# mprib/caliscope

Hardware: AMD Instinct MI355X
Metric: observations/sec per LM iteration (higher is better)
Workload: dtype f64; 1 GPU; cfg4: 64 cams / 2000000 obs in total (200000 points / 2000000 obs on rank 0), extrinsics-only BA, linear loss; n_obs_total=2000000, params_per_camera=6, tolerances=ftol=xtol=gtol=1e-8 (reference defaults), sums=FP64 atomics (default)

## Files before the change

caliscope_amd/csrc/ba_math.h:

```cpp
#pragma once
#include <cstddef>
#include <cmath>
#include <cstdint>

#if defined(__HIPCC__)
#define CBA_HD __host__ __device__ __forceinline__
#else
#define CBA_HD inline
#endif

namespace cba {

constexpr int MODEL_PINHOLE_BC5 = 0;
constexpr int MODEL_FISHEYE4 = 1;
constexpr int CAM_CONST_STRIDE = 12;
constexpr int MAX_NC = 9;
constexpr double EPS_F64 = 2.220446049250313e-16;

CBA_HD double inv_sqrt(double x) {
#if defined(__HIP_DEVICE_COMPILE__)
  double y = __builtin_amdgcn_rsq(x);
  y = y * (1.5 - 0.5 * x * y * y);
  y = y * (1.5 - 0.5 * x * y * y);
  return y;
// ... 134 lines not shown
  const double g10 = fys * L.dyx * iz, g11 = fys * L.dyy * iz;
  const double G[2][3] = {{g00, g01, -(g00 * x + g01 * y)}, {g10, g11, -(g10 * x + g11 * y)}};
  for (int r = 0; r < 2; ++r) {
    A[r][3] = G[r][0]; A[r][4] = G[r][1]; A[r][5] = G[r][2];
    B[r][0] = G[r][0] * c.R[0] + G[r][1] * c.R[3] + G[r][2] * c.R[6];
    B[r][1] = G[r][0] * c.R[1] + G[r][1] * c.R[4] + G[r][2] * c.R[7];
    B[r][2] = G[r][0] * c.R[2] + G[r][1] * c.R[5] + G[r][2] * c.R[8];
  }
  for (int j = 0; j < 3; ++j) {
    const double m0 = c.Jl[j], m1 = c.Jl[3 + j], m2 = c.Jl[6 + j];
    const double c0 = m1 * Y2 - m2 * Y1, c1 = m2 * Y0 - m0 * Y2, c2 = m0 * Y1 - m1 * Y0;
    A[0][j] = G[0][0] * c0 + G[0][1] * c1 + G[0][2] * c2;
    A[1][j] = G[1][0] * c0 + G[1][1] * c1 + G[1][2] * c2;
  }
  if (c.nparams == 9.0) {
    A[0][6] = c.fx0 * L.xd * s; A[1][6] = c.fy0 * L.yd * s;
    A[0][7] = fxs * L.xr2;      A[1][7] = fys * L.yr2;
    A[0][8] = fxs * L.xr4;      A[1][8] = fys * L.yr4;
  }
}

template <bool RES>
CBA_HD void project_factors_impl(const CamTab& c, double X, double Y, double Z, double u, double v,
                                 double* e, double (*G)[3], double* Yr, double (*Aint)[3], double (*B)[3]) {
  const double Y0 = c.R[0] * X + c.R[1] * Y + c.R[2] * Z;
  const double Y1 = c.R[3] * X + c.R[4] * Y + c.R[5] * Z;
  const double Y2 = c.R[6] * X + c.R[7] * Y + c.R[8] * Z;
  Yr[0] = Y0; Yr[1] = Y1; Yr[2] = Y2;
  const double Zc = Y2 + c.t[2];
  const double iz = 1.0 / Zc;
  const double x = (Y0 + c.t[0]) * iz, y = (Y1 + c.t[1]) * iz;
  Lens L;
  if (c.model != 0.0) lens_fisheye(c.d, x, y, &L); else lens_pinhole(c.d, x, y, &L);
  const double s = c.inv_fx0;
  if constexpr (RES) {
    e[0] = ((c.cx - u) + c.fx * L.xd) * s;
    e[1] = ((c.cy - v) + c.fy * L.yd) * s;
  }
  const double fxs = c.fx * s, fys = c.fy * s;
  const double g00 = fxs * L.dxx * iz, g01 = fxs * L.dxy * iz;
  const double g10 = fys * L.dyx * iz, g11 = fys * L.dyy * iz;
  G[0][0] = g00; G[0][1] = g01; G[0][2] = -(g00 * x + g01 * y);
  G[1][0] = g10; G[1][1] = g11; G[1][2] = -(g10 * x + g11 * y);
  for (int r = 0; r < 2; ++r) {
    B[r][0] = G[r][0] * c.R[0] + G[r][1] * c.R[3] + G[r][2] * c.R[6];
    B[r][1] = G[r][0] * c.R[1] + G[r][1] * c.R[4] + G[r][2] * c.R[7];
    B[r][2] = G[r][0] * c.R[2] + G[r][1] * c.R[5] + G[r][2] * c.R[8];
  }
  const bool free_intr = c.nparams == 9.0;
  Aint[0][0] = free_intr ? c.fx0 * L.xd * s : 0.0; Aint[1][0] = free_intr ? c.fy0 * L.yd * s : 0.0;
  Aint[0][1] = free_intr ? fxs * L.xr2 : 0.0;      Aint[1][1] = free_intr ? fys * L.yr2 : 0.0;
  Aint[0][2] = free_intr ? fxs * L.xr4 : 0.0;      Aint[1][2] = free_intr ? fys * L.yr4 : 0.0;
}
CBA_HD void project_factors(const CamTab& c, double X, double Y, double Z, double u, double v,
                            double* e, double (*G)[3], double* Yr, double (*Aint)[3], double (*B)[3]) {
  project_factors_impl<true>(c, X, Y, Z, u, v, e, G, Yr, Aint, B);
}
CBA_HD void project_factors(const CamTab& c, double X, double Y, double Z, double (*G)[3], double* Yr, double (*Aint)[3], double (*B)[3]) {
  project_factors_impl<false>(c, X, Y, Z, 0.0, 0.0, nullptr, G, Yr, Aint, B);
}

CBA_HD double robust_one(int loss, double f_scale, double r, double* row_scale, double* r_scaled) {
  if (loss == LOSS_LINEAR) { *row_scale = 1.0; *r_scaled = r; return r * r; }
  const double fs2 = f_scale * f_scale;
  const double z = (r * r) / fs2;
  double rho0, rho1, rho2;
  switch (loss) {
    case LOSS_HUBER:
      if (z <= 1.0) { rho0 = z; rho1 = 1.0; rho2 = 0.0; }
      else { const double sz = sqrt(z); rho0 = 2.0 * sz - 1.0; rho1 = 1.0 / sz; rho2 = -0.5 / (z * sz); }
      break;
    case LOSS_SOFT_L1: {
      const double t = 1.0 + z, st = sqrt(t);
      rho0 = 2.0 * (st - 1.0); rho1 = 1.0 / st; rho2 = -0.5 / (t * st);
    } break;
    case LOSS_CAUCHY: {
      const double t = 1.0 + z;
      rho0 = log1p(z); rho1 = 1.0 / t; rho2 = -1.0 / (t * t);
    } break;
    default: {
      const double t = 1.0 + z * z;
      rho0 = atan(z); rho1 = 1.0 / t; rho2 = -2.0 * z / (t * t);
// ... 158 lines not shown
```

caliscope_amd/csrc/cba_kernels.h:

```cpp
#pragma once
#include <hip/hip_runtime.h>

#include "ba_math.h"
#include "trf_math.h"
#include "wg_binding.h"
#include "chol_schedule.h"

namespace cba {

constexpr int BLOCK = 256;
constexpr int CHUNK = 256;
constexpr int WAVE = 64;

struct VecLayout {
  int ncp;
  int ncp_pad;
  int P;
  int Ppad;
  __host__ __device__ long total() const { return (long)ncp_pad + 3L * Ppad; }
};

__device__ __forceinline__ double wave_sum(double v) {
#pragma unroll
  for (int o = WAVE / 2; o > 0; o >>= 1) v += __shfl_down(v, o, WAVE);
// ... 290 lines not shown
template <int NC>
__device__ __forceinline__ double obs_linearize(const CamTab& c_lds, double X, double Y, double Z, double u, double v,
                                                int loss, double f_scale, double* e, double (*A)[MAX_NC],
                                                double (*B)[3]) {
  const CamTab c = c_lds;
  __builtin_amdgcn_sched_barrier(0);
  project_full(c, X, Y, Z, u, v, e, A, B);
  double rho = 0.0;
#pragma unroll
  for (int r = 0; r < 2; ++r) {
    double rs, er;
    rho += robust_one(loss, f_scale, e[r], &rs, &er);
    e[r] = er;
    if (loss != LOSS_LINEAR) {
#pragma unroll
      for (int k = 0; k < NC; ++k) A[r][k] *= rs;
      B[r][0] *= rs; B[r][1] *= rs; B[r][2] *= rs;
    }
  }
  return rho;
}

__device__ __forceinline__ double obs_factors(const CamTab& c_lds, double X, double Y, double Z, double u, double v, int loss, double f_scale, double* e,
                                              double (*G)[3], double* Yr, double (*Aint)[3], double (*B)[3]) {
  CamTab c;
  {
    const double* src = reinterpret_cast<const double*>(&c_lds);
    double* dst = reinterpret_cast<double*>(&c);
#pragma unroll
    for (int i = 0; i < 12; ++i) dst[i] = src[i];
#pragma unroll
    for (int i = 21; i < 35; ++i) dst[i] = src[i];
  }
  __builtin_amdgcn_sched_barrier(0);
  project_factors(c, X, Y, Z, u, v, e, G, Yr, Aint, B);
  double rho = 0.0;
#pragma unroll
  for (int r = 0; r < 2; ++r) {
    double rs, er;
    rho += robust_one(loss, f_scale, e[r], &rs, &er);
    e[r] = er;
    if (loss != LOSS_LINEAR) {
#pragma unroll
      for (int k = 0; k < 3; ++k) { G[r][k] *= rs; B[r][k] *= rs; Aint[r][k] *= rs; }
    }
  }
  return rho;
}
__device__ __forceinline__ void obs_factors(const CamTab& c_lds, double X, double Y, double Z, double (*G)[3], double* Yr, double (*Aint)[3], double (*B)[3]) {
  CamTab c;
  {
    const double* src = reinterpret_cast<const double*>(&c_lds);
    double* dst = reinterpret_cast<double*>(&c);
#pragma unroll
    for (int i = 0; i < 12; ++i) dst[i] = src[i];
    dst[21] = src[21]; dst[22] = src[22];
#pragma unroll
    for (int i = 25; i < 35; ++i) dst[i] = src[i];
  }
  __builtin_amdgcn_sched_barrier(0);
  project_factors(c, X, Y, Z, G, Yr, Aint, B);
#pragma unroll
  for (int r = 0; r < 2; ++r) {
#pragma unroll
    for (int k = 0; k < 3; ++k) { asm("" : "+v"(G[r][k])); asm("" : "+v"(B[r][k])); asm("" : "+v"(Aint[r][k])); }
  }
#pragma unroll
  for (int k = 0; k < 3; ++k) asm("" : "+v"(Yr[k]));
}

template <int NC> struct UPack {
  static constexpr int TRI = NC * (NC + 1) / 2;
  static constexpr int STRIDE = TRI + NC;
  __host__ __device__ static constexpr int idx(int r, int c) { return r * NC - r * (r - 1) / 2 + (c - r); }
};

constexpr int DET_ROUND = 9;
constexpr int DET_LD = CHUNK + 1;
struct DetPlan {
  const unsigned char* perm;
  const unsigned short* cstart;
};
template <int M>
__device__ __forceinline__ void det_round(const double* val, double* sh_cv, const int* sh_perm, const int* sh_cs, int n_cams, double* acc) {
#pragma unroll
  for (int q = 0; q < DET_ROUND; ++q) sh_cv[q * DET_LD + threadIdx.x] = val[q];
  __syncthreads();
#pragma unroll
  for (int m = 0; m < M; ++m) {
    const int task = (int)threadIdx.x + BLOCK * m;
    if (task < n_cams * DET_ROUND) {
// ... 585 lines not shown
}

struct TilePlan {
  const int* chunk_start;
  const int* wg_first;
  const int* wg_end;
  const int* wg_tile;
  const int* wg_stride;
  const int* tile_a;
  const int* tile_b;
  const int* group_cam_begin;
  const int* group_par_begin;
  int g;
  int tile_elems;
  const int* obs;
  int rep;
  const unsigned* codes;
  const int* code_start;
  const unsigned* nit;
  int prio_shift;
};

template <int NC> struct SchurRec {
  static constexpr int NVAL = (NC == 9) ? 21 : 12;
  static constexpr int NPH = (NVAL + 1) / 2;
  static constexpr int LST = (NPH & 1) ? NPH : NPH + 1;
  static constexpr int REC = 2 * LST;
  static constexpr int HREC = 2 * NPH;
  static constexpr int STAGE = (HREC / 2) | 1;
  static constexpr int STAGE_WAVES = (NC == 9) ? 2 : 4;
};
static_assert(SchurRec<6>::REC == 14 && SchurRec<6>::LST == 7 && SchurRec<9>::REC == 22 && SchurRec<9>::LST == 11, "record sizes");

template <int NC>
__device__ __forceinline__ void expand_record(const double* __restrict__ rec, const double* __restrict__ Jl, double* __restrict__ T) {
  const double Y0 = rec[0], Y1 = rec[1], Y2 = rec[2];
  const double* Q = rec + 3;
#pragma unroll
  for (int m = 0; m < 3; ++m) {
    const double q0 = Q[m], q1 = Q[3 + m], q2 = Q[6 + m];
    const double c0 = Y1 * q2 - Y2 * q1, c1 = Y2 * q0 - Y0 * q2, c2 = Y0 * q1 - Y1 * q0;
#pragma unroll
    for (int r = 0; r < 3; ++r) T[3 * r + m] = Jl[r] * c0 + Jl[3 + r] * c1 + Jl[6 + r] * c2;
    T[9 + m] = q0; T[12 + m] = q1; T[15 + m] = q2;
  }
  if (NC == 9) {
#pragma unroll
    for (int k = 0; k < 9; ++k) T[18 + k] = rec[12 + k];
  }
}

struct LinFin {
  const double* partial_lin;
  const double* partial_max;
  const double* partial_jv;
  int rows_lin, rows_jv;
  double radius;
  double* scal;
  double* fz;
};
// ... 143 lines not shown
      const int k1 = min(no0 + (int)threadIdx.x, last_obs);
      if constexpr (!LIN) { nx.u = obs_u[k1]; nx.v = obs_v[k1]; }
      nx.cam = obs_cam[k1];
      nn.pt = obs_pt[min(nno0 + (int)threadIdx.x, last_obs)];
    } else {
      nn = load_rec(min((PIPE ? nno0 : no0) + (int)threadIdx.x, last_obs));
    }
    if constexpr (PIPE) __builtin_amdgcn_sched_barrier(0);
    const int i = o0 + threadIdx.x;
    double rec[REC];
#pragma unroll
    for (int k = 0; k < REC; ++k) rec[k] = 0.0;
    double bval[DET_ROUND];
#pragma unroll
    for (int q = 0; q < DET_ROUND; ++q) bval[q] = 0.0;
    if (DET) {
      sh_perm[threadIdx.x] = det.perm[(long)ch * CHUNK + threadIdx.x];
      for (int q = threadIdx.x; q <= n_cams; q += BLOCK) sh_cs[q] = det.cstart[(long)ch * (n_cams + 1) + q];
    }
    if (i < o1) {
      const int cam = cur.cam;
      const CamTab& ct = cam_of<CAMG>(sh_tab, tab, cam);
      const double X = ops.X, Yw = ops.Y, Zw = ops.Z;
      double e[2], G[2][3], Yr[3], Aint[2][3], B[2][3], Z[2][3];
      if constexpr (LIN) obs_factors(ct, X, Yw, Zw, G, Yr, Aint, B);
      else obs_factors(ct, X, Yw, Zw, cur.u, cur.v, loss, f_scale, e, G, Yr, Aint, B);
      const int np = (int)ct.nparams;
      double Vd[6], L[6];
#pragma unroll
      for (int q = 0; q < 6; ++q) Vd[q] = ops.V[q];
      const double d0 = ops.d[0], d1 = ops.d[1], d2 = ops.d[2];
      Vd[0] += lam * d0 * d0; Vd[3] += lam * d1 * d1; Vd[5] += lam * d2 * d2;
      if (!chol3(Vd, L)) {
        fail = true;
        L[0] = L[2] = L[5] = 1.0; L[1] = L[3] = L[4] = 0.0;
      }
      chol3_fwd(L, B[0], Z[0]);
      chol3_fwd(L, B[1], Z[1]);
      const double gpt[3] = {ops.g[0], ops.g[1], ops.g[2]};
      double y[3];
      chol3_fwd(L, gpt, y);
      double* bc = sh_b + (int)ct.pad[0];
      rec[0] = Yr[0]; rec[1] = Yr[1]; rec[2] = Yr[2];
      double qy[3];
#pragma unroll
      for (int r = 3; r < NC; ++r) {
        const bool live = r < np;
        const double a0 = (r < 6) ? G[0][r - 3] : Aint[0][(r - 6) % 3], a1 = (r < 6) ? G[1][r - 3] : Aint[1][(r - 6) % 3];
        double t[3];
#pragma unroll
        for (int k = 0; k < 3; ++k) t[k] = live ? a0 * Z[0][k] + a1 * Z[1][k] : 0.0;
        const double ty = t[0] * y[0] + t[1] * y[1] + t[2] * y[2];
        if (r < 6) qy[r - 3] = ty;
        if (DET) bval[r] = live ? ty : 0.0;
        else if (live) lds_add(&bc[r], ty);
        rec[3 * r - 6] = t[0]; rec[3 * r - 5] = t[1]; rec[3 * r - 4] = t[2];
      }
      {
        const double c0 = Yr[1] * qy[2] - Yr[2] * qy[1], c1 = Yr[2] * qy[0] - Yr[0] * qy[2], c2 = Yr[0] * qy[1] - Yr[1] * qy[0];
        if (DET) {
#pragma unroll
          for (int r = 0; r < 3; ++r) bval[r] = ct.Jl[r] * c0 + ct.Jl[3 + r] * c1 + ct.Jl[6 + r] * c2;
        } else {
          lds_add(&bc[0], c0); lds_add(&bc[1], c1); lds_add(&bc[2], c2);
        }
      }
    }
    if constexpr (PIPE) {
      asm volatile("s_waitcnt vmcnt(0)" ::: "memory");
      if constexpr (FULL) launder_obs(nn); else { launder_obs(nx); asm volatile("" : "+v"(nn.pt)); }
      launder_ops(ops_n);
    }
    const int w0 = o0 + wv * WAVE;
    const int n_pieces = max(0, min(WAVE, o1 - w0)) * NP;
    double2* dst = reinterpret_cast<double2*>(Trec + (long)w0 * REC);
#pragma unroll
    for (int turn = 0; turn < (BLOCK / WAVE) / SW; ++turn) {
      if (wv / SW == turn) {
#pragma unroll
// ... 115 lines not shown
  static constexpr int SPLIT = (NC == 9) ? 3 : 1;
  static constexpr int CODE_THREADS = BLOCK, CODE_WAVES = BLOCK / WAVE;
  static constexpr int REG_BLOCK = BLOCK * SPLIT, NWAVES = REG_BLOCK / WAVE;
  static constexpr int GROUP = 16;
  static constexpr int NCD = (NC == 6) ? 8 : 4;
  static constexpr int PAIR_CAP = 0;
  static constexpr int SCHUNK = (NC == 9) ? 384 : 320;
  static constexpr int EPW = SCHUNK / NWAVES;
  static constexpr int NLD = (EPW * LST + WAVE - 1) / WAVE;
  static constexpr int WAVE_PIECES = NLD * WAVE;
  static constexpr int ZERO_PIECE = NWAVES * WAVE_PIECES;
  static constexpr int BUF_PIECES = ZERO_PIECE + LST + 1;
  static constexpr int NBUF = 2;
  static constexpr int SET_PIECES = NBUF * BUF_PIECES;
  static constexpr bool LANE_TABLE = (NC == 9);
  static constexpr int TABLE_PIECES = LANE_TABLE ? (NLD * WAVE * 4 + 15) / 16 : 0;
  static constexpr size_t LDS_BYTES = (size_t)(SET_PIECES + TABLE_PIECES) * 16;
  static constexpr int LAUNCH_THREADS = REG_BLOCK;
  static_assert(SCHUNK % NWAVES == 0 && EPW % 16 == 0 && EPW <= 2 * WAVE && (LST & 1) == 1, "staging layout");
  static_assert(ZERO_PIECE + LST < 65536, "piece addresses are 16 bit");
  static_assert(CODE_WAVES % 4 == 0, "iteration counts: four waves per word");
};

__device__ __forceinline__ void pair6(double (&acc)[6][6], const double2* __restrict__ Ri, const double2* __restrict__ Rj) {
  const double2 i0 = Ri[0], i1 = Ri[1], i2 = Ri[2], i3 = Ri[3], i4 = Ri[4], i5 = Ri[5];
  const double2 j0 = Rj[0], j1 = Rj[1], j2 = Rj[2], j3 = Rj[3], j4 = Rj[4], j5 = Rj[5];
  const double Yi[3] = {i0.x, i0.y, i1.x}, Yj[3] = {j0.x, j0.y, j1.x};
  const double Qi[9] = {i1.y, i2.x, i2.y, i3.x, i3.y, i4.x, i4.y, i5.x, i5.y};
  const double Qj[9] = {j1.y, j2.x, j2.y, j3.x, j3.y, j4.x, j4.y, j5.x, j5.y};
  double M[3][6];
#pragma unroll
  for (int a = 0; a < 3; ++a) {
#pragma unroll
    for (int b2 = 0; b2 < 3; ++b2)
      M[a][3 + b2] = fma(Qi[3 * a + 2], Qj[3 * b2 + 2], fma(Qi[3 * a + 1], Qj[3 * b2 + 1], Qi[3 * a] * Qj[3 * b2]));
    M[a][0] = fma(Yj[1], M[a][5], -(Yj[2] * M[a][4]));
    M[a][1] = fma(Yj[2], M[a][3], -(Yj[0] * M[a][5]));
    M[a][2] = fma(Yj[0], M[a][4], -(Yj[1] * M[a][3]));
  }
#pragma unroll
  for (int c = 0; c < 6; ++c) {
    acc[0][c] = fma(Yi[1], M[2][c], fma(-Yi[2], M[1][c], acc[0][c]));
    acc[1][c] = fma(Yi[2], M[0][c], fma(-Yi[0], M[2][c], acc[1][c]));
    acc[2][c] = fma(Yi[0], M[1][c], fma(-Yi[1], M[0][c], acc[2][c]));
    acc[3][c] += M[0][c]; acc[4][c] += M[1][c]; acc[5][c] += M[2][c];
  }
}

template <int NC, int RH>
__device__ __forceinline__ void unprime_rows(double (&acc)[RH][NC], int r0, const double* __restrict__ Ji, const double* __restrict__ Jj) {
  if (r0 == 0) {
#pragma unroll
    for (int c = 0; c < NC; ++c) {
      const double b0 = acc[0][c], b1 = acc[1][c], b2 = acc[2][c];
#pragma unroll
      for (int r = 0; r < 3; ++r) acc[r][c] = Ji[r] * b0 + Ji[3 + r] * b1 + Ji[6 + r] * b2;
    }
  }
// ... 32 lines not shown
    for (int c = 0; c < 6; ++c) acc[r][c] = 0.0;

  const int vt = (SPLIT == 1) ? tid : ct;
  const int blk = (rep > 1) ? vt % nblk : vt, slot = (rep > 1) ? vt / nblk : 0;
  const bool owner = slot < rep && blk < nblk;
  double* dst = partial + ((long)wg * rep + min(slot, rep - 1)) * tp.tile_elems + (long)min(blk, nblk - 1) * NC * NC;

  const int stride = tp.wg_stride[wg], ch_end = tp.wg_end[wg];
  const int own_trips = tp.wg_first[wg] < ch_end ? (ch_end - 1 - tp.wg_first[wg]) / stride + 1 : 0;
  const int first = own_trips ? tp.wg_first[wg] : max(ch_end - 1, 0);
  const int trips = max(own_trips, 1);
  for (int k = tid; k < Cfg::NBUF * LST; k += REG_BLOCK) sh_p[(k / LST) * Cfg::BUF_PIECES + Cfg::ZERO_PIECE + k % LST] = make_double2(0.0, 0.0);
  int* const lane_table = reinterpret_cast<int*>(sh_p + Cfg::SET_PIECES);
  if constexpr (Cfg::LANE_TABLE) {
    constexpr int Q = WAVE / LST, RM = WAVE % LST;
    for (int e = tid; e < NLD * WAVE; e += REG_BLOCK) {
      const int k = e / WAVE, l = e % WAVE;
      int piece = k * RM + l % LST;
      const int el = min(k * Q + l / LST + piece / LST, EPW - 1);
      piece = min(piece % LST, SchurRec<NC>::NPH - 1);
      lane_table[e] = el | (piece << 16);
    }
    __syncthreads();
  }
  const int last = first + (own_trips ? (own_trips - 1) * stride : 0);
  struct Raw { unsigned nit[NWORD]; int code_start; int obs_start; };
  auto load_raw = [&](int chunk, int successor) {
    Raw r;
#pragma unroll
    for (int q = 0; q < NWORD; ++q) r.nit[q] = p_nit[(long)chunk * NWORD + q];
    r.code_start = p_code_start[chunk];
    r.obs_start = p_chunk_start[successor];
    return r;
  };
  auto load_indices = [&](int obs_start, int* iA, int* iB) {
    const int* src = p_obs + obs_start + sw * EPW;
    *iA = src[lane];
    if (EPW > WAVE) *iB = src[WAVE + (lane & (EPW - WAVE - 1))];
  };
  static_assert(EPW <= WAVE || ((EPW - WAVE) & (EPW - WAVE - 1)) == 0, "second index register");
  unsigned cd[NCD];
  int n_nx = 0;
  long code_nx = 0;
  auto load_codes = [&](const Raw& r) {
    int pre = 0, mine = 0;
#pragma unroll
// ... 19 lines not shown
      int piece, el;
      if constexpr (Cfg::LANE_TABLE) {
        const int e = lane_table[k * WAVE + lane];
        el = e & 0xffff; piece = e >> 16;
      } else {
        piece = k * RM + lane % LST;
        el = k * Q + lane / LST + piece / LST;
        piece = min(piece % LST, SchurRec<NC>::NPH - 1);
        el = min(el, EPW - 1);
      }
      const bool useB = EPW > WAVE && k * WAVE >= WAVE * LST;
      const int idx = useB ? __shfl(idxB, el - WAVE, WAVE) : __shfl(idxA, el, WAVE);
      g[k] = reinterpret_cast<const double2*>(Trec + (long)idx * SchurRec<NC>::HREC) + piece;
    }
    __builtin_amdgcn_sched_barrier(0);
#pragma unroll
    for (int k = 0; k < NLD; ++k)
      __builtin_amdgcn_global_load_lds((const void __attribute__((address_space(1)))*)g[k], (void __attribute__((address_space(3)))*)(wbase + k * WAVE), 16, 0, 0);
  };
  auto pair = [&](const double2* bufp, unsigned code) {
    const double2* Ri = bufp + (code & 0xffffu);
    const double2* Rj = bufp + (code >> 16);
    if constexpr (NC == 6) {
      pair6(acc, Ri, Rj);
    } else {
      if (half == 0) pair9_corner(acc, Ri, Rj);
      else if (half == 1) pair9_cols(accf, Ri, Rj);
      else pair9_rows(accf, Ri, Rj);
    }
  };

  long long clk_sum[6] = {0, 0, 0, 0, 0, 0};
  const long long t_start = CLK ? clock64() : 0;
  int idxA = 0, idxB = 0;
  const int second = min(first + stride, last);
  Raw raw = load_raw(first, second);
  load_indices(p_chunk_start[first], &idxA, &idxB);
  issue(0, idxA, idxB);
  load_codes(raw);
  load_indices(raw.obs_start, &idxA, &idxB);
  raw = load_raw(second, min(second + stride, last));
  int buf = 0;
  const int young = ((int)blockIdx.x >= (int)gridDim.x / 2) ? 1 : 0;
  for (int trip = 0; trip < trips; ++trip) {
    if (tp.prio_shift >= 0) {
      if (((trip >> tp.prio_shift) + young) & 1) __builtin_amdgcn_s_setprio(1); else __builtin_amdgcn_s_setprio(0);
    }
// ... 26 lines not shown
    __builtin_amdgcn_sched_barrier(0);
    if (CLK) { tD = clock64(); __builtin_amdgcn_sched_barrier(0); }
    const double2* bufp = sh_p + buf * Cfg::BUF_PIECES;
#pragma unroll
    for (int it = 0; it < NCD; ++it)
      if (it < n_cur) pair(bufp, cc[it]);
    for (int it = NCD; it < n_cur; ++it) pair(bufp, p_codes[code_cur + (long)it * WAVE]);
    if (CLK) {
      __builtin_amdgcn_sched_barrier(0);
      const long long tE = clock64();
      clk_sum[0] += tB - tA; clk_sum[1] += tC - tB; clk_sum[2] += tD - tC; clk_sum[3] += tE - tD; clk_sum[4] += 1; clk_sum[5] += n_cur;
    }
    raw = raw_n; idxA = idxA_n; idxB = idxB_n;
    buf ^= 1;
  }
  if (CLK && lane == 0 && clk) {
    long long* o = clk + ((long)wg * Cfg::NWAVES + sw) * 8;
#pragma unroll
    for (int k = 0; k < 6; ++k) o[k] = clk_sum[k];
    o[6] = clock64() - t_start;
    o[7] = ((long long)__builtin_amdgcn_s_getreg((4 << 0) | (0 << 6) | (31 << 11)) << 40) | (wall_clock64() & 0xffffffffffLL);
  }
  asm volatile("s_waitcnt vmcnt(0)" ::: "memory");
  if (blk < nblk) {
    const int tile = tp.wg_tile[wg];
    const int ga = tp.tile_a[tile], gb = tp.tile_b[tile];
    const int ca0 = tp.group_cam_begin[ga], na = tp.group_cam_begin[ga + 1] - ca0;
    const int cb0 = tp.group_cam_begin[gb], nb = tp.group_cam_begin[gb + 1] - cb0;
    const int li = blk / tp.g, lj = blk % tp.g;
    int ci = -1, cj = -1;
    if (ga == gb && lj <= li) {
      const int hk = li * (li + 1) / 2 + lj;
      ci = cj = ca0 + hk % max(na, 1);
    } else if (li < na && lj < nb) {
      ci = ca0 + li; cj = cb0 + lj;
    }
    if (ci >= 0) {
      const double* Ji = tab + (long)ci * CAMTAB_DOUBLES + 12;
      const double* Jj = tab + (long)cj * CAMTAB_DOUBLES + 12;
      if constexpr (NC == 6) {
        unprime_rows<6, 6>(acc, 0, Ji, Jj);
      } else {
        if (half != 2) {
          const double j0 = Ji[0], j1 = Ji[1], j2 = Ji[2], j3 = Ji[3], j4 = Ji[4], j5 = Ji[5], j6 = Ji[6], j7 = Ji[7], j8 = Ji[8];
          if (half == 0) {
#pragma unroll
            for (int c = 0; c < 6; ++c) {
              const double b0 = acc[0][c], b1 = acc[1][c], b2 = acc[2][c];
              acc[0][c] = j0 * b0 + j3 * b1 + j6 * b2; acc[1][c] = j1 * b0 + j4 * b1 + j7 * b2; acc[2][c] = j2 * b0 + j5 * b1 + j8 * b2;
            }
            asm volatile("; role 0 rows" ::: "memory");
          } else {
#pragma unroll
            for (int c = 0; c < 3; ++c) {
              const double b0 = accf[c], b1 = accf[3 + c], b2 = accf[6 + c];
              accf[c] = j0 * b0 + j3 * b1 + j6 * b2; accf[3 + c] = j1 * b0 + j4 * b1 + j7 * b2; accf[6 + c] = j2 * b0 + j5 * b1 + j8 * b2;
            }
            asm volatile("; role 1 rows" ::: "memory");
          }
// ... 1082 lines not shown
        const double g2[3] = {q2[0], q2[1], q2[2]};
        for (int j = a; j < b; ++j) { q2[0] += sh_pt[j]; q2[1] += sh_pt[CHUNK + j]; q2[2] += sh_pt[2 * CHUNK + j]; }
#pragma unroll
        for (int k = 0; k < 6; ++k) V2[k] = Vblk[(long)k * lay.Ppad + p];
#pragma unroll
        for (int k = 0; k < 3; ++k) d2[k] = dp[(long)k * lay.Ppad + p];
        solve_point(p, q2, V2, d2, g2);
      }
    }
    __syncthreads();
    cur = nx; o0 = no0; o1 = no1; ch = nxt;
    pt_next = pt_nn; X = Xn; Yw = Yn; Zw = Zn;
  }
  if (SCAL) {
    double r;
    r = block_sum(sc0, sh_pt); if (threadIdx.x == 0) step_partial[blockIdx.x * 4 + 0] = r;
    r = block_sum(sc1, sh_pt); if (threadIdx.x == 0) { step_partial[blockIdx.x * 4 + 1] = r; step_partial[blockIdx.x * 4 + 2] = 0.0; step_partial[blockIdx.x * 4 + 3] = 0.0; }
  }
}

constexpr int BSR_PT = 3 * CHUNK;
template <int NC> struct BsrCfg {
  static constexpr int NP = SchurRec<NC>::NPH;
  static constexpr int CS = (NC == 9) ? 9 : 6;
  static constexpr int CSS = CS;
  static constexpr size_t lds_bytes(int n_cams) { return ((size_t)BLOCK * NP * 2 + 2 * BSR_PT + (size_t)n_cams * CSS + 8) * sizeof(double); }
};
template <int NC, bool SCAL>
__device__ __forceinline__ void backsub_rec_body(const double* __restrict__ Trec, const int* __restrict__ obs_cam, const int* __restrict__ pt_start,
                                                 const int* __restrict__ chunk_start, const int* __restrict__ chunk_pts, int n_chunks, VecLayout lay,
                                                 const double* __restrict__ tab, const int* __restrict__ cam_off, const int* __restrict__ cam_np,
                                                 int n_cams, double lam, const double* __restrict__ Vblk, const double* __restrict__ gp,
                                                 const double* __restrict__ dp, const double* __restrict__ s_cam, double* __restrict__ sp,
                                                 double* __restrict__ step_partial, double* sh) {
  using Cfg = BsrCfg<NC>;
  constexpr int NP = Cfg::NP, CSS = Cfg::CSS;
  double2* sh_rec = reinterpret_cast<double2*>(sh);
  double* sh_pt = sh + (size_t)BLOCK * NP * 2;
  double* sh_step = sh_pt + 2 * BSR_PT;
  const int tid = (int)threadIdx.x, lane = tid % WAVE;
  const int wv = __builtin_amdgcn_readfirstlane(tid / WAVE);
  for (int idx = tid; idx < n_cams * 3; idx += BLOCK) {
    const int c = idx / 3, a = idx % 3, off = cam_off[c];
    const double* Jl = tab + (long)c * CAMTAB_DOUBLES + 12;
    sh_step[c * CSS + a] = fma(Jl[3 * a + 2], s_cam[off + 2], fma(Jl[3 * a + 1], s_cam[off + 1], Jl[3 * a] * s_cam[off]));
    sh_step[c * CSS + 3 + a] = s_cam[off + 3 + a];
    if (NC == 9) sh_step[c * CSS + 6 + a] = (cam_np[c] == 9) ? s_cam[off + 6 + a] : 0.0;
  }
  const int n_obs = chunk_start[n_chunks];
  const int last_obs = max(n_obs - 1, 0);
  const long last_piece = (long)max(n_obs, 1) * NP - 1;
  const double2* rec_g = reinterpret_cast<const double2*>(Trec);
  double2* wrec = sh_rec + wv * (WAVE * NP);
  auto issue = [&](int o0) {
    const long base = ((long)o0 + wv * WAVE) * NP + lane;
#pragma unroll
    for (int k = 0; k < NP; ++k)
      __builtin_amdgcn_global_load_lds((const void __attribute__((address_space(1)))*)(rec_g + min(base + k * WAVE, last_piece)),
                                       (void __attribute__((address_space(3)))*)(wrec + k * WAVE), 16, 0, 0);
  };
  struct PtIn { int p, a, b, on; double V[6], d[3], g[3]; };
  const int lp0 = lane * 4 + wv;
  auto load_point = [&](int cp0, int npts) {
    PtIn q;
    q.on = lp0 < npts;
    q.p = min(cp0 + min(lp0, max(npts - 1, 0)), lay.P - 1);
    q.a = pt_start[q.p]; q.b = pt_start[q.p + 1];
#pragma unroll
    for (int k = 0; k < 6; ++k) q.V[k] = Vblk[(long)k * lay.Ppad + q.p];
#pragma unroll
// ... 71 lines not shown
#pragma unroll
    for (int k = 0; k < 3; ++k) { asm volatile("" : "+v"(pprev.d[k])); asm volatile("" : "+v"(pprev.g[k])); }
    double2 rec[NP];
    const double2* mine = wrec + lane * NP;
#pragma unroll
    for (int k = 0; k < NP; ++k) rec[k] = mine[k];
    asm volatile("s_waitcnt lgkmcnt(0)" ::: "memory");
#pragma unroll
    for (int k = 0; k < NP; ++k) asm volatile("" : "+v"(rec[k].x), "+v"(rec[k].y));
    const bool more = ch + stride < n_chunks;
    if (more) issue(nx.o0);
    const int ncam = obs_cam[min(nx.o0 + tid, last_obs)];
    const Ent nn = load_ent(min(ch + 2 * stride, last_chunk));
    const PtIn pcur = load_point(cur.cp0, cur.npts);
    __builtin_amdgcn_sched_barrier(0);
    double t0, t1, t2;
    {
      const double* cs = sh_step + cam * CSS;
      const double w0 = cs[0], w1 = cs[1], w2 = cs[2];
      const double Y0 = rec[0].x, Y1 = rec[0].y, Y2 = rec[1].x;
      const double m0 = fma(w1, Y2, fma(-w2, Y1, cs[3]));
      const double m1 = fma(w2, Y0, fma(-w0, Y2, cs[4]));
      const double m2 = fma(w0, Y1, fma(-w1, Y0, cs[5]));
      t0 = fma(rec[4].y, m2, fma(rec[3].x, m1, rec[1].y * m0));
      t1 = fma(rec[5].x, m2, fma(rec[3].y, m1, rec[2].x * m0));
      t2 = fma(rec[5].y, m2, fma(rec[4].x, m1, rec[2].y * m0));
      if constexpr (NC == 9) {
        const double i0 = cs[6], i1 = cs[7], i2 = cs[8];
        t0 = fma(rec[9].x, i2, fma(rec[7].y, i1, fma(rec[6].x, i0, t0)));
        t1 = fma(rec[9].y, i2, fma(rec[8].x, i1, fma(rec[6].y, i0, t1)));
        t2 = fma(rec[10].x, i2, fma(rec[8].y, i1, fma(rec[7].x, i0, t2)));
      }
      if (cur.o0 + tid >= cur.o1) { t0 = 0.0; t1 = 0.0; t2 = 0.0; }
    }
    double* pt = sh_pt + buf * BSR_PT;
    pt[tid] = t0; pt[CHUNK + tid] = t1; pt[2 * CHUNK + tid] = t2;
    point_phase(pprev, sh_pt + (buf ^ 1) * BSR_PT, eprev.cp0, eprev.npts, eprev.o0);
    __syncthreads();
    pprev = pcur; eprev = cur;
    buf ^= 1;
    if (!more) break;
    cam = ncam; cur = nx; nx = nn; ch += stride;
  }
  asm volatile("s_waitcnt vmcnt(0)" ::: "memory");
  point_phase(pprev, sh_pt + (buf ^ 1) * BSR_PT, eprev.cp0, eprev.npts, eprev.o0);
  if (SCAL) {
    __syncthreads();
    double r;
    r = block_sum(sc0, sh_pt); if (tid == 0) step_partial[blockIdx.x * 4 + 0] = r;
// ... 627 lines not shown
  for (int k = 0; k < 3; ++k) q[k] = gp[(long)k * lay.Ppad + p] + sp[(long)k * lay.Ppad + p];
  if (chol3(Vd, L)) { chol3_fwd(L, q, y); chol3_bwd(L, y, x); }
#pragma unroll
  for (int k = 0; k < 3; ++k) sp[(long)k * lay.Ppad + p] = -x[k];
}

template <int NC>
__global__ void __launch_bounds__(BLOCK)
k_heavy_schur(const int* __restrict__ heavy_pts, const int* __restrict__ pt_start, const int* __restrict__ obs_cam,
              const int* __restrict__ cam_off, const int* __restrict__ cam_np, int ncp,
              const double* __restrict__ Trec, const double* __restrict__ tab, double* __restrict__ heavy_W, double* __restrict__ Sacc) {
  constexpr int REC = SchurRec<NC>::HREC;
  extern __shared__ __attribute__((aligned(16))) double sh[];
  double* W = sh;
  int* seen = reinterpret_cast<int*>(W + (size_t)ncp * 3);
  const int h = blockIdx.x, p = heavy_pts[h];
  for (int e = threadIdx.x; e < ncp * 3; e += BLOCK) W[e] = 0.0;
  for (int e = threadIdx.x; e < ncp; e += BLOCK) seen[e] = 0;
  __syncthreads();
  const int o0 = pt_start[p], o1 = pt_start[p + 1];
  for (int i = o0 + threadIdx.x; i < o1; i += BLOCK) {
    const int cam = obs_cam[i], off = cam_off[cam], np = cam_np[cam];
    double T[3 * NC];
    expand_record<NC>(Trec + (long)i * REC, tab + (long)cam * CAMTAB_DOUBLES + 12, T);
#pragma unroll
    for (int r = 0; r < NC; ++r) {
      if (r < np) {
        lds_add(&W[(off + r) * 3 + 0], T[3 * r]); lds_add(&W[(off + r) * 3 + 1], T[3 * r + 1]); lds_add(&W[(off + r) * 3 + 2], T[3 * r + 2]);
        seen[off + r] = 1;
      }
    }
  }
  __syncthreads();
  double* Wg = heavy_W + (long)h * ncp * 3;
  for (int e = threadIdx.x; e < ncp * 3; e += BLOCK) Wg[e] = W[e];
  for (long e = threadIdx.x; e < (long)ncp * ncp; e += BLOCK) {
    const int r = (int)(e / ncp), c = (int)(e % ncp);
    if (c < r || !seen[r] || !seen[c]) continue;
    const double acc = W[r * 3] * W[c * 3] + W[r * 3 + 1] * W[c * 3 + 1] + W[r * 3 + 2] * W[c * 3 + 2];
    unsafeAtomicAdd(&Sacc[(long)r * ncp + c], acc);
  }
}

struct ConPlan {
  int n_con, n_comp;
  const int* pt;
  const int* lp;
// ... 210 lines not shown
    for (int s = 0; s < 8; ++s) {
      const double* z = cp.z + (long)((c0 + c) * 8 + s) * 3;
      const double* y = py + (long)cp.lp[(c0 + c) * 8 + s] * 3;
      h += z[0] * y[0] + z[1] * y[1] + z[2] * y[2];
    }
    G[(long)c * gw + ncp] = h;
    for (int s = 0; s < 8; ++s) {
      const int p = cp.pt[(c0 + c) * 8 + s];
      const double* z = cp.z + (long)((c0 + c) * 8 + s) * 3;
      int hidx = -1;
      for (int lo = 0, hi = cp.n_heavy - 1; lo <= hi;) {
        const int mid = (lo + hi) >> 1, q = cp.heavy_pts[mid];
        if (q == p) { hidx = mid; break; }
        if (q < p) lo = mid + 1; else hi = mid - 1;
      }
      if (hidx >= 0) {
        const double* Wh = cp.heavy_W + (long)hidx * ncp * 3;
        for (int r = 0; r < ncp; ++r) G[(long)c * gw + r] += Wh[3 * r] * z[0] + Wh[3 * r + 1] * z[1] + Wh[3 * r + 2] * z[2];
        continue;
      }
      for (int i = pt_start[p]; i < pt_start[p + 1]; ++i) {
        const int cam = obs_cam[i];
        double T[3 * NC];
        expand_record<NC>(Trec + (long)i * REC, tab + (long)cam * CAMTAB_DOUBLES + 12, T);
        const int off = cam_off[cam], npar = cam_np[cam];
#pragma unroll
        for (int r = 0; r < NC; ++r)
          if (r < npar) G[(long)c * gw + off + r] += T[3 * r] * z[0] + T[3 * r + 1] * z[1] + T[3 * r + 2] * z[2];
      }
    }
  }
  __syncthreads();
  for (int j = 0; j < m; ++j) {
    for (int i = j + threadIdx.x; i < m; i += BLOCK) {
      double v = M[(long)i * m + j];
      for (int t = 0; t < j; ++t) v -= M[(long)i * m + t] * M[(long)j * m + t];
      M[(long)i * m + j] = v;
      if (i == j) sh_piv = v;
    }
    __syncthreads();
    const double piv = sh_piv;
    if (!(piv > 0.0)) { if (threadIdx.x == 0) flags[2] = 1; }
    const double inv = piv > 0.0 ? 1.0 / sqrt(piv) : 1.0;
    for (int i = j + threadIdx.x; i < m; i += BLOCK) M[(long)i * m + j] = (i == j) ? (piv > 0.0 ? sqrt(piv) : 1.0) : M[(long)i * m + j] * inv;
    __syncthreads();
  }
  for (int col = threadIdx.x; col < gw; col += BLOCK) {
// ... 53 lines not shown
#pragma unroll
    for (int q = 0; q < 6; ++q) pL[lp * 6 + q] = L[q];
    py[lp * 3] = y[0]; py[lp * 3 + 1] = y[1]; py[lp * 3 + 2] = y[2];
  }
  for (int e = tid; e < m * ZL; e += BLOCK) Z[e] = 0.0;
  for (int e = tid; e < nz * GW; e += BLOCK) Wst[e] = 0.0;
  __syncthreads();
  for (int e = tid; e < m * 8; e += BLOCK) {
    const int c = c0 + e / 8, sl = e % 8;
    const double q = (sl < 4) ? 0.25 : -0.25;
    const double j3[3] = {q * cp.u[c * 3], q * cp.u[c * 3 + 1], q * cp.u[c * 3 + 2]};
    const int lp = cp.lp[c * 8 + sl];
    double z[3];
    chol3_fwd(pL + lp * 6, j3, z);
    cp.z[(long)(c * 8 + sl) * 3] = z[0]; cp.z[(long)(c * 8 + sl) * 3 + 1] = z[1]; cp.z[(long)(c * 8 + sl) * 3 + 2] = z[2];
    double* zr = Z + (e / 8) * ZL + 3 * lp;
    lds_add(&zr[0], z[0]); lds_add(&zr[1], z[1]); lds_add(&zr[2], z[2]);
  }
  for (int lp = tid / 16; lp < np; lp += BLOCK / 16) {
    const int p = cp.comp_pts[p0 + lp];
    for (int i = pt_start[p] + (tid % 16); i < pt_start[p + 1]; i += 16) {
      const int cam = obs_cam[i];
      double T[3 * NC];
      expand_record<NC>(Trec + (long)i * REC, tab + (long)cam * CAMTAB_DOUBLES + 12, T);
      const int off = cam_off[cam], npar = cam_np[cam];
#pragma unroll
      for (int r = 0; r < NC; ++r)
        if (r < npar) {
          lds_add(&Wst[(3 * lp + 0) * GW + off + r], T[3 * r]);
          lds_add(&Wst[(3 * lp + 1) * GW + off + r], T[3 * r + 1]);
          lds_add(&Wst[(3 * lp + 2) * GW + off + r], T[3 * r + 2]);
        }
    }
  }
  __syncthreads();
  for (int e = tid; e < m * m; e += BLOCK) {
    const int a = e / m, b = e % m;
    const double *za = Z + a * ZL, *zb = Z + b * ZL;
    double acc = (a == b) ? 1.0 : 0.0;
    for (int q = 0; q < nz; ++q) acc = fma(za[q], zb[q], acc);
    M[a * ML + b] = acc;
  }
  for (int e = tid; e < m * gw; e += BLOCK) {
    const int c = e / gw, col = e % gw;
    const double* zc = Z + c * ZL;
    double acc = 0.0;
    if (col < ncp) for (int q = 0; q < nz; ++q) acc = fma(zc[q], Wst[q * GW + col], acc);
// ... 209 lines not shown
```

Measured before the change: 3.984 billion obs/s.

## Compress six-parameter Schur records by storing inverse depth and dropping derived rows

The per-observation Schur record for extrinsics-only cameras shrinks from 14 to 10 doubles. It stores the rotated point, the inverse depth and two rows of the projected Jacobian block, and the third row is rebuilt from the normalized image coordinates using the camera translation. The pair-accumulation, BSR matvec and record-expansion kernels are updated to reconstruct the dropped row on the fly, loading camera translations from the camera table. This cuts memory traffic and LDS footprint for the record stream at the cost of extra FMAs and a few camera-table loads per block.

```diff
diff --git a/caliscope_amd/csrc/ba_math.h b/caliscope_amd/csrc/ba_math.h
--- a/caliscope_amd/csrc/ba_math.h
+++ b/caliscope_amd/csrc/ba_math.h
@@ -180,7 +180,7 @@
 
 template <bool RES>
 CBA_HD void project_factors_impl(const CamTab& c, double X, double Y, double Z, double u, double v,
-                                 double* e, double (*G)[3], double* Yr, double (*Aint)[3], double (*B)[3]) {
+                                 double* e, double (*G)[3], double* Yr, double (*Aint)[3], double (*B)[3], double* nrm = nullptr) {
   const double Y0 = c.R[0] * X + c.R[1] * Y + c.R[2] * Z;
   const double Y1 = c.R[3] * X + c.R[4] * Y + c.R[5] * Z;
   const double Y2 = c.R[6] * X + c.R[7] * Y + c.R[8] * Z;
@@ -188,6 +188,7 @@
   const double Zc = Y2 + c.t[2];
   const double iz = 1.0 / Zc;
   const double x = (Y0 + c.t[0]) * iz, y = (Y1 + c.t[1]) * iz;
+  if (nrm) { nrm[0] = x; nrm[1] = y; nrm[2] = iz; }
   Lens L;
   if (c.model != 0.0) lens_fisheye(c.d, x, y, &L); else lens_pinhole(c.d, x, y, &L);
   const double s = c.inv_fx0;
@@ -211,11 +212,42 @@
   Aint[0][2] = free_intr ? fxs * L.xr4 : 0.0;      Aint[1][2] = free_intr ? fys * L.yr4 : 0.0;
 }
 CBA_HD void project_factors(const CamTab& c, double X, double Y, double Z, double u, double v,
-                            double* e, double (*G)[3], double* Yr, double (*Aint)[3], double (*B)[3]) {
-  project_factors_impl<true>(c, X, Y, Z, u, v, e, G, Yr, Aint, B);
-}
-CBA_HD void project_factors(const CamTab& c, double X, double Y, double Z, double (*G)[3], double* Yr, double (*Aint)[3], double (*B)[3]) {
-  project_factors_impl<false>(c, X, Y, Z, 0.0, 0.0, nullptr, G, Yr, Aint, B);
+                            double* e, double (*G)[3], double* Yr, double (*Aint)[3], double (*B)[3], double* nrm = nullptr) {
+  project_factors_impl<true>(c, X, Y, Z, u, v, e, G, Yr, Aint, B, nrm);
+}
+CBA_HD void project_factors(const CamTab& c, double X, double Y, double Z, double (*G)[3], double* Yr, double (*Aint)[3], double (*B)[3],
+                            double* nrm = nullptr) {
+  project_factors_impl<false>(c, X, Y, Z, 0.0, 0.0, nullptr, G, Yr, Aint, B, nrm);
+}
+
+constexpr int REC6_VALUES = 10;
+CBA_HD void rec6_head(const double* Yr, const double* t, double* nrm) {
+  const double Zc = Yr[2] + t[2];
+  const double iz = 1.0 / Zc;
+  nrm[0] = (Yr[0] + t[0]) * iz; nrm[1] = (Yr[1] + t[1]) * iz; nrm[2] = iz;
+}
+CBA_HD void rec6_pack(const double (*G)[3], const double* Yr, const double (*Z)[3], double iz, double* rec) {
+  rec[0] = Yr[0]; rec[1] = Yr[1]; rec[2] = Yr[2]; rec[3] = iz;
+  for (int r = 0; r < 2; ++r)
+    for (int k = 0; k < 3; ++k) rec[4 + 3 * r + k] = G[0][r] * Z[0][k] + G[1][r] * Z[1][k];
+}
+CBA_HD void rec6_pack(const double (*G)[3], const double* Yr, const double* t, const double (*Z)[3], double* rec) {
+  double nrm[3];
+  rec6_head(Yr, t, nrm);
+  rec6_pack(G, Yr, Z, nrm[2], rec);
+}
+CBA_HD void rec6_xy(const double* rec, const double* t, double* x, double* y) {
+  *x = (rec[0] + t[0]) * rec[3];
+  *y = (rec[1] + t[1]) * rec[3];
+}
+CBA_HD void rec6_expand(const double* rec, const double* t, double* full) {
+  double x, y;
+  rec6_xy(rec, t, &x, &y);
+  full[0] = rec[0]; full[1] = rec[1]; full[2] = rec[2];
+  for (int k = 0; k < 3; ++k) {
+    full[3 + k] = rec[4 + k]; full[6 + k] = rec[7 + k];
+    full[9 + k] = -(x * rec[4 + k] + y * rec[7 + k]);
+  }
 }
 
 CBA_HD double robust_one(int loss, double f_scale, double r, double* row_scale, double* r_scaled) {
diff --git a/caliscope_amd/csrc/cba_kernels.h b/caliscope_amd/csrc/cba_kernels.h
--- a/caliscope_amd/csrc/cba_kernels.h
+++ b/caliscope_amd/csrc/cba_kernels.h
@@ -336,7 +336,7 @@
 }
 
 __device__ __forceinline__ double obs_factors(const CamTab& c_lds, double X, double Y, double Z, double u, double v, int loss, double f_scale, double* e,
-                                              double (*G)[3], double* Yr, double (*Aint)[3], double (*B)[3]) {
+                                              double (*G)[3], double* Yr, double (*Aint)[3], double (*B)[3], double* nrm = nullptr) {
   CamTab c;
   {
     const double* src = reinterpret_cast<const double*>(&c_lds);
@@ -347,7 +347,11 @@
     for (int i = 21; i < 35; ++i) dst[i] = src[i];
   }
   __builtin_amdgcn_sched_barrier(0);
-  project_factors(c, X, Y, Z, u, v, e, G, Yr, Aint, B);
+  project_factors(c, X, Y, Z, u, v, e, G, Yr, Aint, B, nrm);
+  if (nrm) {
+#pragma unroll
+    for (int k = 0; k < 3; ++k) asm("" : "+v"(nrm[k]));
+  }
   double rho = 0.0;
 #pragma unroll
   for (int r = 0; r < 2; ++r) {
@@ -361,7 +365,8 @@
   }
   return rho;
 }
-__device__ __forceinline__ void obs_factors(const CamTab& c_lds, double X, double Y, double Z, double (*G)[3], double* Yr, double (*Aint)[3], double (*B)[3]) {
+__device__ __forceinline__ void obs_factors(const CamTab& c_lds, double X, double Y, double Z, double (*G)[3], double* Yr, double (*Aint)[3], double (*B)[3],
+                                            double* nrm = nullptr) {
   CamTab c;
   {
     const double* src = reinterpret_cast<const double*>(&c_lds);
@@ -373,7 +378,7 @@
     for (int i = 25; i < 35; ++i) dst[i] = src[i];
   }
   __builtin_amdgcn_sched_barrier(0);
-  project_factors(c, X, Y, Z, G, Yr, Aint, B);
+  project_factors(c, X, Y, Z, G, Yr, Aint, B, nrm);
 #pragma unroll
   for (int r = 0; r < 2; ++r) {
 #pragma unroll
@@ -381,6 +386,10 @@
   }
 #pragma unroll
   for (int k = 0; k < 3; ++k) asm("" : "+v"(Yr[k]));
+  if (nrm) {
+#pragma unroll
+    for (int k = 0; k < 3; ++k) asm("" : "+v"(nrm[k]));
+  }
 }
 
 template <int NC> struct UPack {
@@ -1012,7 +1021,7 @@
 };
 
 template <int NC> struct SchurRec {
-  static constexpr int NVAL = (NC == 9) ? 21 : 12;
+  static constexpr int NVAL = (NC == 9) ? 21 : 10;
   static constexpr int NPH = (NVAL + 1) / 2;
   static constexpr int LST = (NPH & 1) ? NPH : NPH + 1;
   static constexpr int REC = 2 * LST;
@@ -1020,12 +1029,17 @@
   static constexpr int STAGE = (HREC / 2) | 1;
   static constexpr int STAGE_WAVES = (NC == 9) ? 2 : 4;
 };
-static_assert(SchurRec<6>::REC == 14 && SchurRec<6>::LST == 7 && SchurRec<9>::REC == 22 && SchurRec<9>::LST == 11, "record sizes");
+static_assert(SchurRec<6>::REC == 10 && SchurRec<6>::LST == 5 && SchurRec<6>::HREC == 10 && SchurRec<6>::STAGE == 5 && SchurRec<9>::REC == 22 &&
+                  SchurRec<9>::LST == 11,
+              "record sizes");
 
 template <int NC>
-__device__ __forceinline__ void expand_record(const double* __restrict__ rec, const double* __restrict__ Jl, double* __restrict__ T) {
-  const double Y0 = rec[0], Y1 = rec[1], Y2 = rec[2];
-  const double* Q = rec + 3;
+__device__ __forceinline__ void expand_record(const double* __restrict__ rec, const double* __restrict__ cam_row, double* __restrict__ T) {
+  const double* Jl = cam_row + 12;
+  double full[12];
+  if constexpr (NC == 6) rec6_expand(rec, cam_row + 9 , full);
+  const double Y0 = (NC == 6) ? full[0] : rec[0], Y1 = (NC == 6) ? full[1] : rec[1], Y2 = (NC == 6) ? full[2] : rec[2];
+  const double* Q = (NC == 6) ? full + 3 : rec + 3;
 #pragma unroll
   for (int m = 0; m < 3; ++m) {
     const double q0 = Q[m], q1 = Q[3 + m], q2 = Q[6 + m];
@@ -1215,9 +1229,9 @@
       const int cam = cur.cam;
       const CamTab& ct = cam_of<CAMG>(sh_tab, tab, cam);
       const double X = ops.X, Yw = ops.Y, Zw = ops.Z;
-      double e[2], G[2][3], Yr[3], Aint[2][3], B[2][3], Z[2][3];
-      if constexpr (LIN) obs_factors(ct, X, Yw, Zw, G, Yr, Aint, B);
-      else obs_factors(ct, X, Yw, Zw, cur.u, cur.v, loss, f_scale, e, G, Yr, Aint, B);
+      double e[2], G[2][3], Yr[3], Aint[2][3], B[2][3], Z[2][3], nrm[3];
+      if constexpr (LIN) obs_factors(ct, X, Yw, Zw, G, Yr, Aint, B, NC == 6 ? nrm : nullptr);
+      else obs_factors(ct, X, Yw, Zw, cur.u, cur.v, loss, f_scale, e, G, Yr, Aint, B, NC == 6 ? nrm : nullptr);
       const int np = (int)ct.nparams;
       double Vd[6], L[6];
 #pragma unroll
@@ -1236,18 +1250,37 @@
       double* bc = sh_b + (int)ct.pad[0];
       rec[0] = Yr[0]; rec[1] = Yr[1]; rec[2] = Yr[2];
       double qy[3];
-#pragma unroll
-      for (int r = 3; r < NC; ++r) {
-        const bool live = r < np;
-        const double a0 = (r < 6) ? G[0][r - 3] : Aint[0][(r - 6) % 3], a1 = (r < 6) ? G[1][r - 3] : Aint[1][(r - 6) % 3];
-        double t[3];
-#pragma unroll
-        for (int k = 0; k < 3; ++k) t[k] = live ? a0 * Z[0][k] + a1 * Z[1][k] : 0.0;
-        const double ty = t[0] * y[0] + t[1] * y[1] + t[2] * y[2];
-        if (r < 6) qy[r - 3] = ty;
-        if (DET) bval[r] = live ? ty : 0.0;
-        else if (live) lds_add(&bc[r], ty);
-        rec[3 * r - 6] = t[0]; rec[3 * r - 5] = t[1]; rec[3 * r - 4] = t[2];
+      if constexpr (NC == 6) {
+        rec[3] = nrm[2];
+#pragma unroll
+        for (int r = 3; r < 5; ++r) {
+          const double a0 = G[0][r - 3], a1 = G[1][r - 3];
+          double t[3];
+#pragma unroll
+          for (int k = 0; k < 3; ++k) t[k] = a0 * Z[0][k] + a1 * Z[1][k];
+          qy[r - 3] = t[0] * y[0] + t[1] * y[1] + t[2] * y[2];
+          rec[3 * r - 5] = t[0]; rec[3 * r - 4] = t[1]; rec[3 * r - 3] = t[2];
+        }
+        qy[2] = -fma(nrm[0], qy[0], nrm[1] * qy[1]);
+#pragma unroll
+        for (int r = 3; r < 6; ++r) {
+          if (DET) bval[r] = qy[r - 3];
+          else lds_add(&bc[r], qy[r - 3]);
+        }
+      } else {
+#pragma unroll
+        for (int r = 3; r < NC; ++r) {
+          const bool live = r < np;
+          const double a0 = (r < 6) ? G[0][r - 3] : Aint[0][(r - 6) % 3], a1 = (r < 6) ? G[1][r - 3] : Aint[1][(r - 6) % 3];
+          double t[3];
+#pragma unroll
+          for (int k = 0; k < 3; ++k) t[k] = live ? a0 * Z[0][k] + a1 * Z[1][k] : 0.0;
+          const double ty = t[0] * y[0] + t[1] * y[1] + t[2] * y[2];
+          if (r < 6) qy[r - 3] = ty;
+          if (DET) bval[r] = live ? ty : 0.0;
+          else if (live) lds_add(&bc[r], ty);
+          rec[3 * r - 6] = t[0]; rec[3 * r - 5] = t[1]; rec[3 * r - 4] = t[2];
+        }
       }
       {
         const double c0 = Yr[1] * qy[2] - Yr[2] * qy[1], c1 = Yr[2] * qy[0] - Yr[0] * qy[2], c2 = Yr[0] * qy[1] - Yr[1] * qy[0];
@@ -1409,18 +1442,33 @@
   static_assert(CODE_WAVES % 4 == 0, "iteration counts: four waves per word");
 };
 
-__device__ __forceinline__ void pair6(double (&acc)[6][6], const double2* __restrict__ Ri, const double2* __restrict__ Rj) {
-  const double2 i0 = Ri[0], i1 = Ri[1], i2 = Ri[2], i3 = Ri[3], i4 = Ri[4], i5 = Ri[5];
-  const double2 j0 = Rj[0], j1 = Rj[1], j2 = Rj[2], j3 = Rj[3], j4 = Rj[4], j5 = Rj[5];
+static_assert(Reg3Cfg<6>::EPW == 80 && Reg3Cfg<6>::LST == 5 && Reg3Cfg<6>::NLD == 7 && Reg3Cfg<6>::WAVE_PIECES == 448 && Reg3Cfg<6>::SCHUNK == 320 &&
+                  Reg3Cfg<6>::ZERO_PIECE == 1792,
+              "six-parameter pair kernel layout");
+
+__device__ __forceinline__ void pair6(double (&acc)[6][6], const double2* __restrict__ Ri, const double2* __restrict__ Rj, double ti0, double ti1, double tj0,
+                                      double tj1) {
+  typedef double piece_t __attribute__((ext_vector_type(2)));
+  const piece_t* Pi = reinterpret_cast<const piece_t*>(Ri);
+  const piece_t* Pj = reinterpret_cast<const piece_t*>(Rj);
+  const piece_t i0 = Pi[0], i1 = Pi[1], i2 = Pi[2], i3 = Pi[3], i4 = Pi[4];
+  const piece_t j0 = Pj[0], j1 = Pj[1], j2 = Pj[2], j3 = Pj[3], j4 = Pj[4];
   const double Yi[3] = {i0.x, i0.y, i1.x}, Yj[3] = {j0.x, j0.y, j1.x};
-  const double Qi[9] = {i1.y, i2.x, i2.y, i3.x, i3.y, i4.x, i4.y, i5.x, i5.y};
-  const double Qj[9] = {j1.y, j2.x, j2.y, j3.x, j3.y, j4.x, j4.y, j5.x, j5.y};
+  const double xi = (Yi[0] + ti0) * i1.y, yi = (Yi[1] + ti1) * i1.y, xj = (Yj[0] + tj0) * j1.y, yj = (Yj[1] + tj1) * j1.y;
+  const double Qi[6] = {i2.x, i2.y, i3.x, i3.y, i4.x, i4.y};
+  const double Qj[6] = {j2.x, j2.y, j3.x, j3.y, j4.x, j4.y};
   double M[3][6];
 #pragma unroll
+  for (int a = 0; a < 2; ++a) {
+#pragma unroll
+    for (int b2 = 0; b2 < 2; ++b2)
+      M[a][3 + b2] = fma(Qi[3 * a + 2], Qj[3 * b2 + 2], fma(Qi[3 * a + 1], Qj[3 * b2 + 1], Qi[3 * a] * Qj[3 * b2]));
+    M[a][5] = -fma(xj, M[a][3], yj * M[a][4]);
+  }
+#pragma unroll
+  for (int b2 = 0; b2 < 3; ++b2) M[2][3 + b2] = -fma(xi, M[0][3 + b2], yi * M[1][3 + b2]);
+#pragma unroll
   for (int a = 0; a < 3; ++a) {
-#pragma unroll
-    for (int b2 = 0; b2 < 3; ++b2)
-      M[a][3 + b2] = fma(Qi[3 * a + 2], Qj[3 * b2 + 2], fma(Qi[3 * a + 1], Qj[3 * b2 + 1], Qi[3 * a] * Qj[3 * b2]));
     M[a][0] = fma(Yj[1], M[a][5], -(Yj[2] * M[a][4]));
     M[a][1] = fma(Yj[2], M[a][3], -(Yj[0] * M[a][5]));
     M[a][2] = fma(Yj[0], M[a][4], -(Yj[1] * M[a][3]));
@@ -1499,6 +1547,31 @@
       lane_table[e] = el | (piece << 16);
     }
     __syncthreads();
+  }
+  int ci = -1, cj = -1;
+  auto block_cameras = [&]() {
+    if (blk >= nblk) return;
+    const int tile = tp.wg_tile[wg];
+    const int ga = tp.tile_a[tile], gb = tp.tile_b[tile];
+    const int ca0 = tp.group_cam_begin[ga], na = tp.group_cam_begin[ga + 1] - ca0;
+    const int cb0 = tp.group_cam_begin[gb], nb = tp.group_cam_begin[gb + 1] - cb0;
+    const int li = blk / tp.g, lj = blk % tp.g;
+    if (ga == gb && lj <= li) {
+      const int hk = li * (li + 1) / 2 + lj;
+      ci = cj = ca0 + hk % max(na, 1);
+    } else if (li < na && lj < nb) {
+      ci = ca0 + li; cj = cb0 + lj;
+    }
+  };
+  double ti0 = 0.0, ti1 = 0.0, tj0 = 0.0, tj1 = 0.0;
+  if constexpr (NC == 6) {
+    block_cameras();
+    if (ci >= 0) {
+      ti0 = tab[(long)ci * CAMTAB_DOUBLES + 9]; ti1 = tab[(long)ci * CAMTAB_DOUBLES + 10];
+      tj0 = tab[(long)cj * CAMTAB_DOUBLES + 9]; tj1 = tab[(long)cj * CAMTAB_DOUBLES + 10];
+    }
+    asm volatile("s_waitcnt vmcnt(0)" ::: "memory");
+    asm volatile("" : "+v"(ti0), "+v"(ti1), "+v"(tj0), "+v"(tj1));
   }
   const int last = first + (own_trips ? (own_trips - 1) * stride : 0);
   struct Raw { unsigned nit[NWORD]; int code_start; int obs_start; };
@@ -1564,7 +1637,7 @@
     const double2* Ri = bufp + (code & 0xffffu);
     const double2* Rj = bufp + (code >> 16);
     if constexpr (NC == 6) {
-      pair6(acc, Ri, Rj);
+      pair6(acc, Ri, Rj, ti0, ti1, tj0, tj1);
     } else {
       if (half == 0) pair9_corner(acc, Ri, Rj);
       else if (half == 1) pair9_cols(accf, Ri, Rj);
@@ -1637,19 +1710,8 @@
     o[7] = ((long long)__builtin_amdgcn_s_getreg((4 << 0) | (0 << 6) | (31 << 11)) << 40) | (wall_clock64() & 0xffffffffffLL);
   }
   asm volatile("s_waitcnt vmcnt(0)" ::: "memory");
-  if (blk < nblk) {
-    const int tile = tp.wg_tile[wg];
-    const int ga = tp.tile_a[tile], gb = tp.tile_b[tile];
-    const int ca0 = tp.group_cam_begin[ga], na = tp.group_cam_begin[ga + 1] - ca0;
-    const int cb0 = tp.group_cam_begin[gb], nb = tp.group_cam_begin[gb + 1] - cb0;
-    const int li = blk / tp.g, lj = blk % tp.g;
-    int ci = -1, cj = -1;
-    if (ga == gb && lj <= li) {
-      const int hk = li * (li + 1) / 2 + lj;
-      ci = cj = ca0 + hk % max(na, 1);
-    } else if (li < na && lj < nb) {
-      ci = ca0 + li; cj = cb0 + lj;
-    }
+  {
+    if constexpr (NC != 6) block_cameras();
     if (ci >= 0) {
       const double* Ji = tab + (long)ci * CAMTAB_DOUBLES + 12;
       const double* Jj = tab + (long)cj * CAMTAB_DOUBLES + 12;
@@ -2778,7 +2840,7 @@
 constexpr int BSR_PT = 3 * CHUNK;
 template <int NC> struct BsrCfg {
   static constexpr int NP = SchurRec<NC>::NPH;
-  static constexpr int CS = (NC == 9) ? 9 : 6;
+  static constexpr int CS = (NC == 9) ? 9 : 8;
   static constexpr int CSS = CS;
   static constexpr size_t lds_bytes(int n_cams) { return ((size_t)BLOCK * NP * 2 + 2 * BSR_PT + (size_t)n_cams * CSS + 8) * sizeof(double); }
 };
@@ -2802,6 +2864,7 @@
     sh_step[c * CSS + a] = fma(Jl[3 * a + 2], s_cam[off + 2], fma(Jl[3 * a + 1], s_cam[off + 1], Jl[3 * a] * s_cam[off]));
     sh_step[c * CSS + 3 + a] = s_cam[off + 3 + a];
     if (NC == 9) sh_step[c * CSS + 6 + a] = (cam_np[c] == 9) ? s_cam[off + 6 + a] : 0.0;
+    if (NC == 6 && a < 2) sh_step[c * CSS + 6 + a] = tab[(long)c * CAMTAB_DOUBLES + 9 + a];
   }
   const int n_obs = chunk_start[n_chunks];
   const int last_obs = max(n_obs - 1, 0);
@@ -2919,9 +2982,17 @@
       const double m0 = fma(w1, Y2, fma(-w2, Y1, cs[3]));
       const double m1 = fma(w2, Y0, fma(-w0, Y2, cs[4]));
       const double m2 = fma(w0, Y1, fma(-w1, Y0, cs[5]));
-      t0 = fma(rec[4].y, m2, fma(rec[3].x, m1, rec[1].y * m0));
-      t1 = fma(rec[5].x, m2, fma(rec[3].y, m1, rec[2].x * m0));
-      t2 = fma(rec[5].y, m2, fma(rec[4].x, m1, rec[2].y * m0));
+      if constexpr (NC == 6) {
+        const double x = (Y0 + cs[6]) * rec[1].y, y = (Y1 + cs[7]) * rec[1].y;
+        const double v0 = fma(-x, m2, m0), v1 = fma(-y, m2, m1);
+        t0 = fma(rec[3].y, v1, rec[2].x * v0);
+        t1 = fma(rec[4].x, v1, rec[2].y * v0);
+        t2 = fma(rec[4].y, v1, rec[3].x * v0);
+      } else {
+        t0 = fma(rec[4].y, m2, fma(rec[3].x, m1, rec[1].y * m0));
+        t1 = fma(rec[5].x, m2, fma(rec[3].y, m1, rec[2].x * m0));
+        t2 = fma(rec[5].y, m2, fma(rec[4].x, m1, rec[2].y * m0));
+      }
       if constexpr (NC == 9) {
         const double i0 = cs[6], i1 = cs[7], i2 = cs[8];
         t0 = fma(rec[9].x, i2, fma(rec[7].y, i1, fma(rec[6].x, i0, t0)));
@@ -3595,7 +3666,7 @@
   for (int i = o0 + threadIdx.x; i < o1; i += BLOCK) {
     const int cam = obs_cam[i], off = cam_off[cam], np = cam_np[cam];
     double T[3 * NC];
-    expand_record<NC>(Trec + (long)i * REC, tab + (long)cam * CAMTAB_DOUBLES + 12, T);
+    expand_record<NC>(Trec + (long)i * REC, tab + (long)cam * CAMTAB_DOUBLES, T);
 #pragma unroll
     for (int r = 0; r < NC; ++r) {
       if (r < np) {
@@ -3852,7 +3923,7 @@
       for (int i = pt_start[p]; i < pt_start[p + 1]; ++i) {
         const int cam = obs_cam[i];
         double T[3 * NC];
-        expand_record<NC>(Trec + (long)i * REC, tab + (long)cam * CAMTAB_DOUBLES + 12, T);
+        expand_record<NC>(Trec + (long)i * REC, tab + (long)cam * CAMTAB_DOUBLES, T);
         const int off = cam_off[cam], npar = cam_np[cam];
 #pragma unroll
         for (int r = 0; r < NC; ++r)
@@ -3952,7 +4023,7 @@
     for (int i = pt_start[p] + (tid % 16); i < pt_start[p + 1]; i += 16) {
       const int cam = obs_cam[i];
       double T[3 * NC];
-      expand_record<NC>(Trec + (long)i * REC, tab + (long)cam * CAMTAB_DOUBLES + 12, T);
+      expand_record<NC>(Trec + (long)i * REC, tab + (long)cam * CAMTAB_DOUBLES, T);
       const int off = cam_off[cam], npar = cam_np[cam];
 #pragma unroll
       for (int r = 0; r < NC; ++r)
```

After: 4.139 billion obs/s, median of 6. 1.04x the previous value.
